# AI-Unicamp/interspeech_ser

Hardware: AMD Instinct MI355X
Metric: utterances/sec (10 s @16 kHz) WavLM-large embed extract (higher is better)
Workload: dtype bf16; 1 GPU; microsoft/wavlm-large embed extract, batch=16 x 10 s @16 kHz per GPU, all 25 hidden states to HBM, mode=bf16; a counted step = 8 such batches (128 utterances per GPU), 2 in flight at a time; batch=16, batches_in_flight=2, frames_per_utt=499, parallelism=utterance-sharded x1, no collective (one process)

## Files before the change

### interspeech_ser_amd/csrc/gemm.hip

```cpp
#include "ser_common.h"
#include "launch_plan.h"
#ifndef SER_GEMM_PP
#define SER_GEMM_PP 27
#endif
#include <stdlib.h>
#include <stdio.h>
#include <utility>
#ifdef SER_GEMM_DBG
extern "C" { void* ser_gemm_dbg_ptr = nullptr; }
__device__ unsigned long long* ser_gemm_dbg_dev = nullptr;
#endif

typedef const __attribute__((address_space(1))) void* gptr_t;
typedef __attribute__((address_space(3))) void* lptr_t;

__device__ __forceinline__ const char* uniform_ptr(const void* p) {
    const uint64_t v = (uint64_t)p;
    const uint32_t lo = __builtin_amdgcn_readfirstlane((uint32_t)v), hi = __builtin_amdgcn_readfirstlane((uint32_t)(v >> 32));
    return (const char*)(((uint64_t)hi << 32) | lo);
}
template <int BYTES>
__device__ __forceinline__ void dma_lds(const void* ubase, uint32_t voff, uint32_t lds_addr) {
    static_assert(BYTES == 16 || BYTES == 4, "dwordx4 or dword");
    if constexpr (BYTES == 16)
        asm volatile("s_mov_b32 m0, %2\n\tglobal_load_lds_dwordx4 %0, %1" :: "v"(voff), "s"(ubase), "s"(lds_addr) : "memory");
    else
        asm volatile("s_mov_b32 m0, %2\n\tglobal_load_lds_dword %0, %1" :: "v"(voff), "s"(ubase), "s"(lds_addr) : "memory");
}

template <int N>
__device__ __forceinline__ void wait_vmcnt() {
    if constexpr (N == 0) asm volatile("s_waitcnt vmcnt(0)" ::: "memory");
    else if constexpr (N == 1) asm volatile("s_waitcnt vmcnt(1)" ::: "memory");
    else if constexpr (N == 2) asm volatile("s_waitcnt vmcnt(2)" ::: "memory");
    else if constexpr (N == 3) asm volatile("s_waitcnt vmcnt(3)" ::: "memory");
    else if constexpr (N == 4) asm volatile("s_waitcnt vmcnt(4)" ::: "memory");
    else if constexpr (N == 5) asm volatile("s_waitcnt vmcnt(5)" ::: "memory");
    else if constexpr (N == 6) asm volatile("s_waitcnt vmcnt(6)" ::: "memory");
    else if constexpr (N == 7) asm volatile("s_waitcnt vmcnt(7)" ::: "memory");
    else if constexpr (N == 8) asm volatile("s_waitcnt vmcnt(8)" ::: "memory");
    else if constexpr (N == 10) asm volatile("s_waitcnt vmcnt(10)" ::: "memory");
    else if constexpr (N == 12) asm volatile("s_waitcnt vmcnt(12)" ::: "memory");
    else if constexpr (N == 16) asm volatile("s_waitcnt vmcnt(16)" ::: "memory");
    else static_assert(N < 0, "add a case");
}

__device__ __forceinline__ void mfma_scale8(f32x4& acc, const i32x8& a, const i32x8& b, int sa, int sb) {
    asm volatile("v_mfma_scale_f32_16x16x128_f8f6f4 %0, %1, %2, %0, %3, %4 op_sel_hi:[0,0,0]" : "+v"(acc) : "v"(a), "v"(b), "v"(sa), "v"(sb));
}
__device__ __forceinline__ void mfma_scale_drain() {
    asm volatile("s_nop 15\n\ts_nop 15\n\ts_nop 7" ::: "memory");
}

template <int WM, int WN, int TM, int TN, int BK, int ST, int MODE, bool LNEPI, int OM = MODE>
__global__ __launch_bounds__(64 * WM * WN, 2)
void ser_gemm_kernel(const ser_gemm_args p) {
    constexpr int NW = WM * WN, NT = 64 * NW;
    constexpr int BM = WM * TM * 16, BN = WN * TN * 16;
    constexpr int CH = BK / 8;
    constexpr int ROWB = BK * 2;
    constexpr int RPP = 1024 / ROWB;
    constexpr bool M16 = (MODE == SER_MODE_FP16M);
    constexpr int NPL = M16 ? 1 : mode_traits<MODE>::planes;
    constexpr int A_BYTES = BM * ROWB, W_BYTES = BN * ROWB, STAGE = NPL * (A_BYTES + W_BYTES);
    static_assert(!M16 || (BK == 64 && !LNEPI && (BM + BN) % 64 == 0), "FP16M: 64-deep K tiles, dense epilogue");
    constexpr int SCW = BM + BN;
    constexpr int LA = BM / RPP / NW, LW = BN / RPP / NW;
    constexpr int LPT = NPL * (LA + LW);
    constexpr int KS = BK / 32;
    static_assert(BM % (RPP * NW) == 0 && BN % (RPP * NW) == 0, "tile/wave mismatch");
    extern __shared__ __attribute__((aligned(16))) char lds[];

    const int tid = threadIdx.x;
    const int lane = tid & 63;
    const int wave = __builtin_amdgcn_readfirstlane(tid >> 6);
    const int wm = wave / WN, wn = wave % WN;
#ifdef SER_GEMM_DBG
    const unsigned long long dbg_e0 = __builtin_amdgcn_s_memtime();
#endif

    const int ntn = (p.N + BN - 1) / BN;
    const int ntm = (p.M + BM - 1) / BM;
    int bid = blockIdx.x;
    {
        const int nwg = ntm * ntn;
        const int q = nwg >> 3, r = nwg & 7, xcd = bid & 7;
        const int base = (xcd < r) ? xcd * (q + 1) : r * (q + 1) + (xcd - r) * q;
        bid = base + (bid >> 3);
    }
    const int mt = bid / ntn;
    const int nt = bid - mt * ntn;
    const int g = blockIdx.y;
    const int m0 = mt * BM, n0 = nt * BN;

    const unsigned short* Abase = (const unsigned short*)p.A + (int64_t)g * p.a_group_stride;
    const unsigned short* Wbase = (const unsigned short*)p.W + (int64_t)g * p.w_group_stride;

    const int prow = lane / CH, ppos = lane % CH;
    uint32_t aoff[LA], woff[LW];
    const int m0c = m0 < p.M ? m0 : p.M - 1;
    const int64_t arow0 = p.a_rowoff ? (int64_t)p.a_rowoff[m0c] * 8 : (int64_t)m0c * p.lda;
    const char* const Atile = uniform_ptr(Abase + arow0);
    const char* const Wtile = uniform_ptr(Wbase + (int64_t)n0 * p.K);
#pragma unroll
    for (int q = 0; q < LA; ++q) {
        const int R = (q * NW + wave) * RPP + prow;
        const int f = (BK == 64) ? (R & 7) : ((R >> 1) & 3);
        const int c = ppos ^ f;
        int m = m0 + R;
        m = m < p.M ? m : p.M - 1;
        const int64_t arow = p.a_rowoff ? (int64_t)p.a_rowoff[m] * 8 : (int64_t)m * p.lda;
        aoff[q] = (uint32_t)((arow - arow0 + c * 8) * 2);
    }
#pragma unroll
    for (int q = 0; q < LW; ++q) {
        const int R = (q * NW + wave) * RPP + prow;
        const int f = (BK == 64) ? (R & 7) : ((R >> 1) & 3);
        const int c = ppos ^ f;
        int n = n0 + R;
        n = n < p.N ? n : p.N - 1;
        woff[q] = (uint32_t)(((int64_t)(n - n0) * p.K + c * 8) * 2);
    }
    const uint32_t lds0 = __builtin_amdgcn_readfirstlane((uint32_t)(uintptr_t)(__attribute__((address_space(3))) char*)lds);

    const int nk = p.K / BK;
    const int total = M16 ? 2 * nk : nk;
    const int tpc = p.kc ? p.kc / BK : 0x7fffffff;

    unsigned char* const scl = (unsigned char*)(lds + ST * STAGE + (LNEPI ? 0 : BM * 8));
    const int sc_chunk = M16 ? (wave % (SCW / 64)) : 0;
    const bool sc_is_a = sc_chunk * 64 < BM;
    const char* const sc_base = uniform_ptr(sc_is_a ? p.a_scale : p.w_scale);
    const int64_t sc_step = (sc_is_a ? p.a_scale_ld : p.w_scale_ld) * 4;
    uint32_t sc_off = 0;
    if constexpr (M16) {
        const int r = sc_chunk * 64 + lane;
        int i = sc_is_a ? m0 + r : n0 + r - BM;
        const int lim = sc_is_a ? p.M : p.N;
        i = i < lim ? i : lim - 1;
        sc_off = (uint32_t)i * 4u;
    }
    int i_kk = 0, i_cc = 0, i_cj = 0, i_stage = 0;
    const char* is_ua = nullptr; const char* is_uw = nullptr;
    uint32_t is_dstA = 0, is_dstW = 0;
    auto issue_begin = [&]() {
        int64_t koffA = (int64_t)i_cj * p.ldj + (int64_t)i_cc * BK;
        int64_t koffW = (int64_t)i_kk * BK;
        if constexpr (M16) {
// ... 440 lines not shown
    if constexpr (LNEPI) {
        __syncthreads();
        float* red = (float*)lds;
        const float invN = 1.0f / (float)p.N;
        float mean[TM], rstd[TM], nmr[TM];
#pragma unroll
        for (int mi = 0; mi < TM; ++mi) {
            float s1 = 0.f, s2 = 0.f;
#pragma unroll
            for (int ni = 0; ni < TN; ++ni)
#pragma unroll
                for (int r = 0; r < 4; ++r) {
                    const float x = acc[ni][mi][r] + bias[ni * 4 + r];
                    acc[ni][mi][r] = x;
                    if (ncol0 + ni * 16 < p.N) { s1 += x; s2 += x * x; }
                }
            s1 += __shfl_xor(s1, 16, 64); s2 += __shfl_xor(s2, 16, 64);
            s1 += __shfl_xor(s1, 32, 64); s2 += __shfl_xor(s2, 32, 64);
            if (fq == 0) {
                red[((wm * TM * 16 + mi * 16 + frow) * WN + wn) * 2] = s1;
                red[((wm * TM * 16 + mi * 16 + frow) * WN + wn) * 2 + 1] = s2;
            }
        }
        __syncthreads();
#pragma unroll
        for (int mi = 0; mi < TM; ++mi) {
            float s1 = 0.f, s2 = 0.f;
#pragma unroll
            for (int w = 0; w < WN; ++w) {
                s1 += red[((wm * TM * 16 + mi * 16 + frow) * WN + w) * 2];
                s2 += red[((wm * TM * 16 + mi * 16 + frow) * WN + w) * 2 + 1];
            }
            mean[mi] = s1 * invN;
            rstd[mi] = rsqrtf(fmaxf(s2 * invN - mean[mi] * mean[mi], 0.f) + p.ln_eps);
            nmr[mi] = -mean[mi] * rstd[mi];
        }
        float lg[CPL], lb[CPL];
#pragma unroll
        for (int j4 = 0; j4 < TN; ++j4) {
            f32x4 a = {0.f, 0.f, 0.f, 0.f}, b = {0.f, 0.f, 0.f, 0.f};
            if (ncol0 + j4 * 16 < p.N) {
                a = *(const f32x4*)(p.ln_gamma + ncol0 + j4 * 16);
                b = *(const f32x4*)(p.ln_beta + ncol0 + j4 * 16);
            }
#pragma unroll
            for (int r = 0; r < 4; ++r) { lg[j4 * 4 + r] = a[r]; lb[j4 * 4 + r] = b[r]; }
        }
#pragma unroll
        for (int mi = 0; mi < TM; ++mi) {
            const int m = m0 + wm * TM * 16 + mi * 16 + frow;
            if (m >= p.M) continue;
            const int64_t orow = p.out_rowmap ? (int64_t)p.out_rowmap[m] : (int64_t)m;
#pragma unroll
            for (int ni = 0; ni < TN; ni += 2) {
                const bool ok0 = ncol0 + ni * 16 < p.N, ok1 = ncol0 + ni * 16 + 16 < p.N;
                float v[8];
#pragma unroll
                for (int r = 0; r < 8; ++r) {
                    const int nj = ni + (r >> 2), rr = r & 3;
                    v[r] = fmaf(fmaf(acc[nj][mi][rr], rstd[mi], nmr[mi]), lg[nj * 4 + rr], lb[nj * 4 + rr]);
                }
                if (p.act == SER_ACT_GELU) {
#pragma unroll
                    for (int r = 0; r < 8; r += 2) {
                        const f32x2 y = gelu2<MODE == SER_MODE_BF16>((f32x2){v[r], v[r + 1]});
                        v[r] = y[0]; v[r + 1] = y[1];
                    }
                }
                if (p.out_f32) {
                    f32x4 o0 = {v[0], v[1], v[2], v[3]}, o1 = {v[4], v[5], v[6], v[7]};
                    if (ok0) *(f32x4*)(p.out_f32 + (int64_t)m * p.ldo_f32 + gcol + ni * 16) = o0;
                    if (ok1) *(f32x4*)(p.out_f32 + (int64_t)m * p.ldo_f32 + gcol + ni * 16 + 16) = o1;
                }
                if (p.out_act) {
                    const int c8 = ni * 16 + ((fq & 1) ? 12 : 0);
                    store_act8_swap<MODE>((unsigned short*)p.out_act + orow * p.ldo_act + gcol + c8, p.out_plane_stride,
                                          ncol0 + c8 < p.N, v);
                    if constexpr (mode_traits<MODE>::f16) {
                        if (p.range_flag) range_fold8(ramax, v, ok0, ok1);
                    }
                }
            }
        }
    } else {
        const bool do_scale = p.col_scale_end > 0;
        const bool do_stat = p.stat_out != nullptr;
        float cs[TM];
#pragma unroll
        for (int mi = 0; mi < TM; ++mi) {
            cs[mi] = 0.f;
            if (p.shift_out) {
                int m = m0 + wm * TM * 16 + mi * 16 + frow;
                m = m < p.M ? m : p.M - 1;
                cs[mi] = p.shift_const + (p.shift_in ? p.shift_in[m] : 0.f);
            }
        }
        constexpr int RB = (TM * TN > 16) ? 2 : (TM < 4 ? TM : 4);
        f32x4 rres[RB][TN];
#pragma unroll
        for (int mi = 0; mi < TM; ++mi) {
            if (mi % RB == 0 && p.residual) {
#pragma unroll
                for (int u = 0; u < RB; ++u) {
                    int mr = m0 + wm * TM * 16 + (mi + u) * 16 + frow;
                    mr = mr < p.M ? mr : p.M - 1;
                    const int rr_ = p.res_row_mod ? (mr % p.res_row_mod) : mr;
#pragma unroll
                    for (int ni = 0; ni < TN; ++ni) {
                        f32x4 r = {0.f, 0.f, 0.f, 0.f};
                        if (ncol0 + ni * 16 < p.N) r = *(const f32x4*)(p.residual + (int64_t)rr_ * p.ldr + gcol + ni * 16);
                        rres[u][ni] = r;
                    }
                }
            }
            const int m = m0 + wm * TM * 16 + mi * 16 + frow;
            if (m >= p.M) continue;
            const int64_t orow = p.out_rowmap ? (int64_t)p.out_rowmap[m] : (int64_t)m;
            float mu = 0.f, rs = 1.f;
            if (p.ln_stats_in) {
                mu = lnst[2 * (wm * TM * 16 + mi * 16 + frow)];
                rs = lnst[2 * (wm * TM * 16 + mi * 16 + frow) + 1];
            }
            const float cshift = cs[mi];
            if (p.shift_out && nt == 0 && g == 0 && wn == 0 && fq == 0) p.shift_out[m] = cshift;
            const float* gsc = nullptr;
            const float* gsh = nullptr;
            if (p.gn_scale) {
                int lo = 0, hi = p.gn_B;
                while (hi - lo > 1) { const int mid = (lo + hi) >> 1; if (p.gn_row_offs[mid] <= m) lo = mid; else hi = mid; }
                gsc = p.gn_scale + (int64_t)lo * p.gn_ld + ncol0;
                gsh = p.gn_shift + (int64_t)lo * p.gn_ld + ncol0;
            }
            float st1 = 0.f, st2 = 0.f;
            unsigned mcode[2] = {0u, 0u};
#pragma unroll
            for (int ni = 0; ni < TN; ni += 2) {
                const bool ok0 = ncol0 + ni * 16 < p.N, ok1 = ncol0 + ni * 16 + 16 < p.N;
                float v[8];
#pragma unroll
                for (int r = 0; r < 8; ++r) {
                    const int nj = ni + (r >> 2), rr = r & 3;
                    float x = fmaf(rs, acc[nj][mi][rr] - mu * csum[nj * 4 + rr], bias[nj * 4 + rr]);
                    if (gsc && ncol0 + nj * 16 < p.N) x = fmaf(x, gsc[nj * 16 + rr], gsh[nj * 16 + rr]);
                    if (do_scale && ncol0 + nj * 16 < p.col_scale_end) x *= p.col_scale;
                    v[r] = x;
                }
                if (p.act == SER_ACT_GELU) {
#pragma unroll
                    for (int r = 0; r < 8; r += 2) {
                        const f32x2 y = gelu2<MODE == SER_MODE_BF16>((f32x2){v[r], v[r + 1]});
                        v[r] = y[0]; v[r + 1] = y[1];
                    }
                }
                if (p.residual) {
                    const f32x4 r0 = rres[mi % RB][ni], r1 = rres[mi % RB][ni + 1];
                    v[0] += r0[0]; v[1] += r0[1]; v[2] += r0[2]; v[3] += r0[3];
                    v[4] += r1[0]; v[5] += r1[1]; v[6] += r1[2]; v[7] += r1[3];
                }
                if (p.out_f32) {
                    float* op = p.out_f32 + (int64_t)m * p.ldo_f32 + gcol + ni * 16 - p.f32_col_begin;
                    f32x4 o0 = {v[0], v[1], v[2], v[3]}, o1 = {v[4], v[5], v[6], v[7]};
                    if (ok0 && ncol0 + ni * 16 >= p.f32_col_begin) *(f32x4*)op = o0;
                    if (ok1 && ncol0 + ni * 16 + 16 >= p.f32_col_begin) *(f32x4*)(op + 16) = o1;
                }
                if (p.shift_out) {
#pragma unroll
                    for (int r = 0; r < 8; ++r) v[r] -= cshift;
                }
                if (do_stat && ok0) {
#pragma unroll
                    for (int r = 0; r < 4; ++r) { st1 += v[r]; st2 += v[r] * v[r]; }
                }
                if (do_stat && ok1) {
#pragma unroll
                    for (int r = 4; r < 8; ++r) { st1 += v[r]; st2 += v[r] * v[r]; }
                }
                if (p.out_act) {
                    const int c8 = ni * 16 + ((fq & 1) ? 12 : 0);
                    if constexpr (OM == SER_MODE_FP16M) {
                        store_act8_swap<SER_MODE_FP16>((unsigned short*)p.out_act + orow * p.ldo_act + gcol + c8, 0, ncol0 + c8 < p.N, v);
                        float lo[8], ax = 0.f, al = 0.f;
#pragma unroll
                        for (int r = 0; r < 8; r += 2) {
                            const unsigned h2 = pack_h2(v[r], v[r + 1]);
                            lo[r] = v[r] - h2f((unsigned short)(h2 & 0xffffu));
                            lo[r + 1] = v[r + 1] - h2f((unsigned short)(h2 >> 16));
                            ax = fmaxf(ax, fmaxf(fabsf(v[r]), fabsf(v[r + 1])));
                            al = fmaxf(al, fmaxf(fabsf(lo[r]), fabsf(lo[r + 1])));
                        }
                        if (p.range_flag) range_fold8(ramax, v, ok0, ok1);
                        ax = max_rowquad(ax); al = max_rowquad(al);
                        const unsigned cx = mx_code(ax), cl = mx_code(al);
                        const float ix = mx_inv(cx), il = mx_inv(cl);
                        unsigned q4[4] = {mx_pack4(lo[0] * il, lo[1] * il, lo[2] * il, lo[3] * il), mx_pack4(lo[4] * il, lo[5] * il, lo[6] * il, lo[7] * il),
                                          mx_pack4(v[0] * ix, v[1] * ix, v[2] * ix, v[3] * ix), mx_pack4(v[4] * ix, v[5] * ix, v[6] * ix, v[7] * ix)};
                        transpose_rowquad(q4);
                        const int64_t bcol = gcol - fq * 4 + ni * 16;
                        unsigned char* seg = (unsigned char*)((unsigned short*)p.out_act + p.out_plane_stride) + (orow * p.ldo_act + (bcol & ~(int64_t)63)) * 2;
                        if (ok0) *(u32x4*)(seg + (fq >> 1) * 64 + (bcol & 63) + (fq & 1) * 16) = (u32x4){q4[0], q4[1], q4[2], q4[3]};
                        mcode[(ni >> 1) & 1] = cl | (cx << 16);
                        if (((ni >> 1) & 1) && fq == 0 && ok0)
                            p.out_scale[(bcol >> 6) * p.out_scale_ld + orow] = (mcode[0] & 0xffu) | ((mcode[1] & 0xffu) << 8) | (mcode[0] & 0xff0000u) | ((mcode[1] & 0xff0000u) << 8);
                    } else {
                        store_act8_swap<OM>((unsigned short*)p.out_act + orow * p.ldo_act + gcol + c8, p.out_plane_stride,
                                            ncol0 + c8 < p.N, v);
                        if constexpr (mode_traits<OM>::f16) {
                            if (p.range_flag) range_fold8(ramax, v, ok0, ok1);
                        }
                    }
                }
            }
            if (p.stat_out) {
                st1 += __shfl_xor(st1, 16, 64); st2 += __shfl_xor(st2, 16, 64);
                st1 += __shfl_xor(st1, 32, 64); st2 += __shfl_xor(st2, 32, 64);
                const int cstart = n0 + wn * (TN * 16);
                const int grp = g * ((p.N + 63) >> 6) + (cstart >> 6);
                if (fq == 0 && cstart < p.N && grp < p.stat_groups) {
                    float* d = p.stat_out + ((int64_t)m * p.stat_groups + grp) * 2;
                    d[0] = st1; d[1] = st2;
                    if constexpr (TN * 16 > 64) {
                        if (cstart + 64 < p.N) { d[2] = 0.f; d[3] = 0.f; }
                    }
                }
            }
        }
    }
    if constexpr (mode_traits<OM>::f16) range_report(p.range_flag, ramax);
#ifdef SER_GEMM_DBG
    {
        __builtin_amdgcn_sched_barrier(0);
        asm volatile("s_waitcnt vmcnt(0)" ::: "memory");
        const unsigned long long t2 = __builtin_amdgcn_s_memtime();
        unsigned long long* d = ser_gemm_dbg_dev;
        if (d && wave == 0 && lane == 0 && blockIdx.y == 0) d[131072 + blockIdx.x * 4 + 2] = t2;
    }
#endif
}

template <int... I, class F>
static bool with_index(int i, std::integer_sequence<int, I...>, F&& f) { return ser_with_mode<I...>(i, f); }

template <int TILE, int PAIR>
static int launch_planned(const ser_gemm_args* a, const gemm_launch& pl, hipStream_t s) {
    constexpr gemm_tile t = GEMM_TILE[TILE];
    constexpr gemm_pair pr = GEMM_PAIR[PAIR];
    auto k = ser_gemm_kernel<t.WM, t.WN, t.TM, t.TN, t.BK, t.ST, pr.mode, t.LNEPI, pr.om>;
    static std::atomic<bool> ready{false};
    if (pl.lds > 65536)
        if (hipError_t e = ser_lds_optin(k, pl.lds, ready)) return ser_fail((int)e, "ser_gemm: cannot raise dynamic LDS to %d", pl.lds);
    hipLaunchKernelGGL(k, dim3(pl.grid_x, pl.grid_y, 1), dim3((unsigned)pl.block, 1, 1), pl.lds, s, *a);
    return ser_check_launch("ser_gemm");
}

extern "C" int ser_gemm(const ser_gemm_args* a, void* stream) {
    gemm_launch pl;
    if (int rc = gemm_plan(a, &pl)) return rc;
    hipStream_t s = (hipStream_t)stream;
#ifdef SER_GEMM_DBG
    {
        static void* planted = nullptr;
        if (planted != ser_gemm_dbg_ptr) {
            planted = ser_gemm_dbg_ptr;
            (void)hipMemcpyToSymbol(HIP_SYMBOL(ser_gemm_dbg_dev), &planted, sizeof(void*));
        }
    }
#endif
    int rc = -22;
    with_index(pl.tile, std::make_integer_sequence<int, GEMM_TILES>{}, [&](auto T) {
        with_index(pl.pair, std::make_integer_sequence<int, GEMM_PAIRS>{}, [&](auto P) {
            constexpr int tile = decltype(T)::value, pair = decltype(P)::value;
            if constexpr (gemm_tile_serves(GEMM_TILE[tile], GEMM_PAIR[pair])) rc = launch_planned<tile, pair>(a, pl, s);
        });
    });
    return rc;
}
```

### interspeech_ser_amd/csrc/launch_plan.h

```cpp
#pragma once
#include <stddef.h>
#include <stdint.h>
#include <stdio.h>
#include <stdlib.h>
#include "../../include/ser_hip.h"

int ser_fail(int code, const char* fmt, ...);

#ifdef SER_EXPERIMENTS
static inline long ser_knob(const char* name, long dflt) { const char* e = getenv(name); return e ? atol(e) : dflt; }
#else
constexpr long ser_knob(const char*, long dflt) { return dflt; }
#endif

struct gemm_tile {
    const char* name;
    int WM, WN, TM, TN, BK, ST;
    bool LNEPI, two_plane;
    constexpr int BM() const { return WM * TM * 16; }
    constexpr int BN() const { return WN * TN * 16; }
    constexpr int threads() const { return 64 * WM * WN; }
    constexpr bool dense() const { return !LNEPI && BN() >= 128; }
};
enum gemm_tile_id {
// ... 33 lines not shown
constexpr int GEMM_PAIRS = (int)(sizeof(GEMM_PAIR) / sizeof(GEMM_PAIR[0]));
constexpr int gemm_pair_index(int mode, int om) {
    for (int i = 0; i < GEMM_PAIRS; ++i)
        if (GEMM_PAIR[i].mode == mode && GEMM_PAIR[i].om == om) return i;
    return -1;
}
constexpr bool gemm_two_plane(int mode) { return mode == SER_MODE_FP32X || mode == SER_MODE_FP16X; }
constexpr bool gemm_tile_serves(const gemm_tile& t, gemm_pair p) {
    if (t.two_plane != gemm_two_plane(p.mode)) return false;
    if (p.mode == SER_MODE_FP16M) return t.dense() && t.BK == 64;
    if (p.om == p.mode) return true;
    if (t.two_plane && p.om == SER_MODE_FP16) return !t.LNEPI;
    return t.dense();
}

struct gemm_knobs {
    int ln_bm, n64, deepk;
    long t256_min, x32_256_min, x32_sq_min, m16_sq_min, m16_256_min;
};
static inline const gemm_knobs& gemm_knobs_get() {
    static const gemm_knobs k = {
        (int)ser_knob("SER_GEMM_LN_BM", 0), (int)ser_knob("SER_GEMM_N64", 1), (int)ser_knob("SER_GEMM_DEEPK_256x128", 1),
        ser_knob("SER_GEMM_T256_MIN", 150),
        ser_knob("SER_GEMM_X32_256_MIN", 100),
        ser_knob("SER_GEMM_X32_SQ_MIN", 150), ser_knob("SER_GEMM_M16_SQ_MIN", 100), ser_knob("SER_GEMM_M16_256_MIN", 100)};
    return k;
}

#ifdef SER_EXPERIMENTS
static inline int gemm_forced_tile(const ser_gemm_args* a) {
    struct Rule { int n, k, cfg; };
    static Rule rules[8];
    static const int nrules = [] {
        const char* e = getenv("SER_GEMM_FORCE");
        int n = 0;
        while (e && *e && n < 8) {
            int a0, a1, a2, used = 0;
            if (sscanf(e, "%d:%d:%d%n", &a0, &a1, &a2, &used) != 3) break;
            rules[n++] = {a0, a1, a2};
            e += used;
            if (*e == ',') ++e;
        }
        return n;
    }();
    for (int i = 0; i < nrules; ++i)
        if (rules[i].n == a->N && rules[i].k == a->K && rules[i].cfg >= 0 && rules[i].cfg <= GEMM_256x256) return rules[i].cfg;
    return -1;
}
#endif

static inline int gemm_pick_tile(const ser_gemm_args* a) {
    const gemm_knobs& kn = gemm_knobs_get();
    const long rt256 = (a->M + 255) / 256;
    const long t256sq = rt256 * ((a->N + 255) / 256) * a->groups;
    const long t256x128 = rt256 * ((a->N + 127) / 128) * a->groups;
    if (gemm_two_plane(a->mode)) {
        if (a->ln_gamma) return GEMM_X_LN128x512x32;
        if (kn.n64 && a->N <= 64) return GEMM_X_128x64x32;
        const long sq_rounds = (t256sq + 255) / 256;
        const bool sq_full = t256sq * 100 >= sq_rounds * 256 * 85;
        if (kn.x32_sq_min > 0 && a->N >= 256 && t256sq >= kn.x32_sq_min && sq_full && a->act == SER_ACT_NONE) return GEMM_X_256x256x32;
        if (kn.x32_256_min > 0 && a->N >= 128 && t256x128 >= kn.x32_256_min) return GEMM_X_256x128x32;
        return GEMM_X_128x128x64;
    }
    if (a->mode == SER_MODE_FP16M) {
        if (a->tile_cfg == 3 || (!a->tile_cfg && a->N >= 256 && t256sq >= kn.m16_sq_min)) return GEMM_256x256;
        if (a->tile_cfg == 2 || (!a->tile_cfg && a->N >= 128 && t256x128 >= kn.m16_256_min)) return GEMM_256x128;
        return GEMM_128x128;
    }
    if (a->ln_gamma) {
        const int bm = kn.ln_bm ? kn.ln_bm : (a->M >= 200 * 128 ? 128 : (a->M >= 200 * 64 ? 64 : 32));
        return bm == 128 ? GEMM_LN512 : (bm == 64 ? GEMM_LN512_M64 : GEMM_LN512_M32);
    }
    if (a->tile_cfg > 0) return a->tile_cfg - 1;
#ifdef SER_EXPERIMENTS
    if (const int forced = gemm_forced_tile(a); forced >= 0) return forced;
#endif
    if (a->N >= 256 && t256sq >= kn.t256_min) return GEMM_256x256;
    if (kn.n64 && a->N <= 64) return GEMM_128x64;
    if (kn.deepk && a->groups == 1 && a->K >= 2048 && a->N >= 128 && a->M >= 512) return GEMM_256x128;
    return GEMM_128x128;
}

struct gemm_launch {
    int tile, pair;
    unsigned grid_x, grid_y;
    int block, lds;
};

static inline int gemm_plan(const ser_gemm_args* a, gemm_launch* out) {
    if (!a || !a->A || !a->W) return ser_fail(-1, "ser_gemm: null operand");
    if (a->M <= 0 || a->N <= 0 || a->K <= 0) return ser_fail(-2, "ser_gemm: bad shape M=%d N=%d K=%d", a->M, a->N, a->K);
    if (a->K % 64) return ser_fail(-3, "ser_gemm: K=%d must be a multiple of 64", a->K);
    if (a->kc && (a->kc % 64 || a->K % a->kc)) return ser_fail(-4, "ser_gemm: kc=%d must divide K and be a multiple of 64", a->kc);
    if (a->N % 8) return ser_fail(-5, "ser_gemm: N=%d must be a multiple of 8", a->N);
    if (gemm_pair_index(a->mode, a->mode) < 0) return ser_fail(-6, "ser_gemm: bad mode %d", a->mode);
    if (a->mode == SER_MODE_FP16M) {
        if (!a->a_scale || !a->w_scale || a->a_scale_ld < a->M || a->w_scale_ld < a->N)
            return ser_fail(-23, "ser_gemm: FP16M needs a_scale / w_scale with *_scale_ld >= the row count");
        if (a->a_rowoff || a->kc || a->groups != 1 || a->ln_gamma || (a->lda % 64))
            return ser_fail(-23, "ser_gemm: FP16M takes plain row-major operands (no row map / conv chunks / groups / LayerNorm epilogue), lda %% 64 == 0");
    }
    if (a->out_mode == SER_MODE_FP16M || (a->mode == SER_MODE_FP16M && !a->out_mode && a->out_act)) {
        if (!a->out_scale || (a->N % 64) || (a->ldo_act % 64) || a->groups != 1 || a->ln_gamma)
            return ser_fail(-24, "ser_gemm: an FP16M out_act needs out_scale, N %% 64 == 0, ldo_act %% 64 == 0, groups == 1, no LayerNorm epilogue");
    }
    if (!a->a_rowoff && (a->lda % 8)) return ser_fail(-7, "ser_gemm: lda must be a multiple of 8");
    if (a->groups < 1) return ser_fail(-8, "ser_gemm: groups=%d", a->groups);
    if (!a->out_f32 && !a->out_act) return ser_fail(-9, "ser_gemm: no output");
    if ((a->ldo_f32 % 4) || (a->ldo_act % 4) || (a->ldr % 4) || (a->c_group_stride % 4))
        return ser_fail(-10, "ser_gemm: output/residual pitches must be multiples of 4");
    if (a->ln_gamma) {
        if (!a->ln_beta) return ser_fail(-11, "ser_gemm: ln_gamma without ln_beta");
        if (a->N > 512 || a->groups != 1 || a->residual)
            return ser_fail(-12, "ser_gemm: the LayerNorm epilogue needs N <= 512, groups == 1, no residual");
    }
    if (a->ln_stats_in) {
        if (!a->ln_colsum || a->ln_groups < 2 || a->ln_groups > 32 || (a->ln_groups & 1) || a->ln_gamma)
            return ser_fail(-14, "ser_gemm: deferred LayerNorm needs ln_colsum, an even ln_groups in [2,32] and no fused-LN epilogue");
    }
    if (a->stat_out && (a->ln_gamma || a->stat_groups < a->groups * ((a->N + 63) / 64)))
        return ser_fail(-15, "ser_gemm: stat_out needs stat_groups >= groups*ceil(N/64) and no fused-LN epilogue");
    if (a->shift_out && (!a->stat_out || a->ln_gamma)) return ser_fail(-19, "ser_gemm: shift_out needs stat_out and no fused-LN epilogue");
    if (a->mean_out && !a->ln_stats_in) return ser_fail(-20, "ser_gemm: mean_out needs ln_stats_in");
    if (a->lnstat_out && !a->ln_stats_in) return ser_fail(-20, "ser_gemm: lnstat_out needs ln_stats_in");
    const int om = a->out_mode ? a->out_mode : a->mode;
    const int pair = gemm_pair_index(a->mode, om);
    if (om != a->mode && !a->ln_gamma && pair < 0)
        return ser_fail(-21, "ser_gemm: out_mode %d with mode %d (FP32X -> FP16, FP16 <-> FP16X, FP16X <-> FP16M convert)", a->out_mode, a->mode);
    if (om != a->mode && a->ln_gamma) return ser_fail(-21, "ser_gemm: out_mode %d with the LayerNorm epilogue", a->out_mode);
    if (a->col_scale_end % 4) return ser_fail(-17, "ser_gemm: col_scale_end must be a multiple of 4");
    if (a->gn_scale && (!a->gn_shift || !a->gn_row_offs || a->gn_B < 1 || a->gn_ld < a->N || (a->gn_ld % 4) || a->groups != 1 ||
                        a->ln_gamma || a->ln_stats_in))
        return ser_fail(-25, "ser_gemm: gn_scale needs gn_shift, gn_row_offs, gn_B >= 1, gn_ld >= N (multiple of 4), groups == 1, "
                             "no LayerNorm epilogue and no deferred LayerNorm");
    if ((a->ldo_act % 8) || (a->c_group_stride % 8)) return ser_fail(-18, "ser_gemm: act pitch / group stride must be multiples of 8");
    if (a->f32_col_begin < 0 || (a->f32_col_begin % 8)) return ser_fail(-16, "ser_gemm: f32_col_begin must be a non-negative multiple of 8");
    if (a->tile_cfg < 0 || a->tile_cfg > 3) return ser_fail(-13, "ser_gemm: tile_cfg=%d (0 auto, 1..3)", a->tile_cfg);

    const int tile = gemm_pick_tile(a);
    const gemm_tile& t = GEMM_TILE[tile];
    if (!gemm_tile_serves(t, GEMM_PAIR[pair])) {
        if (a->mode == SER_MODE_FP16M) return ser_fail(-22, "ser_gemm: FP16M needs a dense tile (N > 64, no LayerNorm epilogue)");
        if (a->mode == SER_MODE_FP16X) return ser_fail(-22, "ser_gemm: FP16X -> FP16M output needs a dense tile (N > 64)");
        return ser_fail(-22, "ser_gemm: FP16 -> FP16X output needs a dense tile (N > 64, no LayerNorm epilogue)");
    }
    const int BM = t.BM(), BN = t.BN();
    out->tile = tile;
    out->pair = pair;
    out->grid_x = (unsigned)(((a->M + BM - 1) / BM) * ((a->N + BN - 1) / BN));
    out->grid_y = (unsigned)a->groups;
    out->block = t.threads();
    out->lds = (gemm_two_plane(a->mode) ? 2 : 1) * t.ST * (BM + BN) * t.BK * 2 + (t.LNEPI ? 0 : BM * 8)
             + (a->mode == SER_MODE_FP16M ? t.ST * (BM + BN) * 4 : 0);
    return 0;
}

constexpr int ATTN_BKV = 64;
constexpr int ATTN_NWV = 4;

struct attn_launch {
    int dhp, mode;
    bool pre, tbl, b2d, gb, occ;
    int nbuf, bias_stride;
    size_t lds;
    int nq;
    unsigned grid;
};
constexpr int attn_qk_planes(int mode) { return (mode == SER_MODE_FP32X || mode == SER_MODE_FP16X || mode == SER_MODE_FP16Q) ? 2 : 1; }
constexpr int attn_v_planes(int mode) { return (mode == SER_MODE_FP32X || mode == SER_MODE_FP16X) ? 2 : 1; }
constexpr bool attn_form_built(int dhp, int mode, bool pre, bool tbl, bool b2d, bool gb, bool occ) {
    if (b2d) return dhp == 64 && pre && !tbl && !gb && !occ && (mode == SER_MODE_BF16 || mode == SER_MODE_FP32X || mode == SER_MODE_FP16X);
    if (gb) return dhp == 64 && pre && tbl && !occ;
    if (occ) return dhp == 64 && attn_qk_planes(mode) == 1;
    return pre || (mode != SER_MODE_FP16X && mode != SER_MODE_FP16Q);
}

static inline int attn_plan(const ser_attention_args* a, attn_launch* out) {
    if (!a) return ser_fail(-1, "ser_attention: null pointer");
    if (!a->qkv || !a->frame_offs || !a->out) return ser_fail(-1, "ser_attention: null pointer");
    const int np = attn_qk_planes(a->mode), npv = attn_v_planes(a->mode);
    if (a->gate_x) {
        if (!a->table || !a->gru_const || a->gate || !a->gate_stat || !a->gate_w || !a->gate_cb)
            return ser_fail(-13, "ser_attention: gate_x needs table, gru_const, gate_stat, gate_w, gate_cb and no gate[]");
        if ((a->gate_x_ld % 8) || (a->gate_x_plane_stride % 8) || (a->gate_w_plane_stride % 8) || a->gate_x_planes != np || (a->dh % 8))
            return ser_fail(-13, "ser_attention: gate_x / gate_w pitch, or gate_x_planes != the planes of mode %d", a->mode);
    }
    if (a->out_mode && a->out_mode != SER_MODE_FP16M) return ser_fail(-14, "ser_attention: out_mode %d (0 or SER_MODE_FP16M)", a->out_mode);
    if (a->out_mode == SER_MODE_FP16M &&
        (a->mode != SER_MODE_FP16X || a->dh != 64 || !a->out_scale || (a->ldo % 64) || a->bias2d || a->out_scale_ld <= 0))
        return ser_fail(-14, "ser_attention: SER_MODE_FP16M context rows need mode FP16X, head dim 64, out_scale, ldo %% 64 == 0 and no bias2d");
    if (a->B <= 0 || a->H <= 0 || a->max_frames <= 0) return ser_fail(-2, "ser_attention: bad B/H/max_frames");
    if (a->dh % 8 || a->dh < 8 || a->dh > 128) return ser_fail(-3, "ser_attention: head dim %d unsupported (multiple of 8, <= 128)", a->dh);
    if ((a->ld % 8) || (a->ldo % 4) || (a->q_col % 8) || (a->k_col % 8) || (a->v_col % 8)) return ser_fail(-4, "ser_attention: misaligned pitches/columns");
    if (a->mode < SER_MODE_BF16 || a->mode > SER_MODE_FP16Q) return ser_fail(-5, "ser_attention: bad mode %d", a->mode);
    if ((a->table != nullptr) != (a->gate != nullptr || a->gru_const != nullptr))
        return ser_fail(-6, "ser_attention: the bias table needs a gate (gate[] or gate_col + gru_const) and vice versa");
    if (a->gate && a->gru_const) return ser_fail(-9, "ser_attention: give gate[] or gru_const, not both");
    if (a->gru_const && !a->gate_x && (a->gate_col < 0 || (a->gate_col % 2))) return ser_fail(-10, "ser_attention: bad gate_col %d", a->gate_col);
    if (a->table && a->table_T < a->max_frames) return ser_fail(-7, "ser_attention: bias table built for T=%d < max_frames=%d", a->table_T, a->max_frames);
    const bool pre = a->scale <= 0.f;
    if (a->bias2d) {
        if (a->table || !a->key_lens || !pre || a->dh > 64 || a->mode == SER_MODE_FP16 || a->mode == SER_MODE_FP16Q)
            return ser_fail(-11, "ser_attention: bias2d needs key_lens, a pre-scaled q (scale <= 0), dh <= 64, no table, bf16 / fp32x / fp16x");
        if (a->bias2d_ld < a->max_frames || (a->bias2d_ld % ATTN_BKV))
            return ser_fail(-12, "ser_attention: bias2d_ld=%lld must be a multiple of %d and >= max_frames", (long long)a->bias2d_ld, ATTN_BKV);
    }
    const int dhp = a->dh <= 64 ? 64 : (a->dh <= 96 ? 96 : 128);
    const int nch = ATTN_BKV * (dhp / 8) / (64 * ATTN_NWV);
    const int nq = (a->max_frames + 32 * ATTN_NWV - 1) / (32 * ATTN_NWV);
    const unsigned nblocks = (unsigned)(((a->H * a->B + 7) / 8) * 8 * nq);
    int bias_stride = 0;
    if (a->table) {
        bias_stride = ((a->max_frames + 32 * ATTN_NWV + 2 * ATTN_BKV + 3 + 4) / 4) * 4;
        bias_stride += (16 - (bias_stride & 63) + 64) & 63;
    }
    const auto nbuf_of = [&](bool occ_) { return (!occ_ && nch * (np + npv) <= 8) ? 2 : 1; };
    const auto lds_of = [&](int nbuf_) { return (size_t)nbuf_ * (np + npv) * ATTN_BKV * dhp * 2 + (size_t)4 * bias_stride * 4; };
    bool occ = dhp == 64 && np == 1 && !a->bias2d && nblocks > 2u * 256u && nblocks <= 4u * 256u;
    int nbuf = nbuf_of(occ);
    size_t lds = lds_of(nbuf);
    if (occ && lds > 40 * 1024) {
        occ = false;
        nbuf = nbuf_of(occ);
        lds = lds_of(nbuf);
    }
    const bool gb = a->table && lds > 160 * 1024 && pre && dhp == 64 && ATTN_NWV == 4;
    if (gb) {
        occ = false;
        nbuf = nbuf_of(occ);
        bias_stride = 0;
        lds = lds_of(nbuf);
// ... 8 lines not shown
```

### interspeech_ser_amd/csrc/launch_plan_check.cc

```cpp
#include "launch_plan.h"
#include <string.h>
#include <iostream>
#include <sstream>
#include <string>

enum kind { I32, I64, F32, PTR };
struct field { const char* name; size_t off; kind k; };
#define F(S, M, K) {#M, offsetof(S, M), K}
static const field GEMM_FIELDS[] = {
    F(ser_gemm_args, A, PTR), F(ser_gemm_args, a_rowoff, PTR), F(ser_gemm_args, lda, I64), F(ser_gemm_args, kc, I32), F(ser_gemm_args, W, PTR),
    F(ser_gemm_args, M, I32), F(ser_gemm_args, N, I32), F(ser_gemm_args, K, I32), F(ser_gemm_args, groups, I32),
    F(ser_gemm_args, c_group_stride, I32), F(ser_gemm_args, mode, I32), F(ser_gemm_args, act, I32), F(ser_gemm_args, residual, PTR),
    F(ser_gemm_args, ldr, I64), F(ser_gemm_args, out_f32, PTR), F(ser_gemm_args, ldo_f32, I64), F(ser_gemm_args, out_act, PTR),
    F(ser_gemm_args, ldo_act, I64), F(ser_gemm_args, ln_gamma, PTR), F(ser_gemm_args, ln_beta, PTR), F(ser_gemm_args, tile_cfg, I32),
    F(ser_gemm_args, ln_stats_in, PTR), F(ser_gemm_args, ln_groups, I32), F(ser_gemm_args, ln_colsum, PTR), F(ser_gemm_args, stat_out, PTR),
    F(ser_gemm_args, stat_groups, I32), F(ser_gemm_args, f32_col_begin, I32), F(ser_gemm_args, col_scale_end, I32),
    F(ser_gemm_args, shift_out, PTR), F(ser_gemm_args, out_mode, I32), F(ser_gemm_args, mean_out, PTR), F(ser_gemm_args, lnstat_out, PTR),
    F(ser_gemm_args, a_scale, PTR), F(ser_gemm_args, a_scale_ld, I64), F(ser_gemm_args, w_scale, PTR), F(ser_gemm_args, w_scale_ld, I64),
    F(ser_gemm_args, out_scale, PTR), F(ser_gemm_args, gn_scale, PTR), F(ser_gemm_args, gn_shift, PTR), F(ser_gemm_args, gn_row_offs, PTR),
    F(ser_gemm_args, gn_B, I32), F(ser_gemm_args, gn_ld, I32),
};
static const field ATTN_FIELDS[] = {
    F(ser_attention_args, qkv, PTR), F(ser_attention_args, ld, I64), F(ser_attention_args, q_col, I32), F(ser_attention_args, k_col, I32),
    F(ser_attention_args, v_col, I32), F(ser_attention_args, B, I32), F(ser_attention_args, frame_offs, PTR), F(ser_attention_args, table, PTR),
    F(ser_attention_args, gate, PTR), F(ser_attention_args, max_frames, I32), F(ser_attention_args, table_T, I32), F(ser_attention_args, out, PTR),
    F(ser_attention_args, ldo, I64), F(ser_attention_args, H, I32), F(ser_attention_args, dh, I32), F(ser_attention_args, scale, F32),
    F(ser_attention_args, mode, I32), F(ser_attention_args, gate_col, I32), F(ser_attention_args, out_mode, I32),
    F(ser_attention_args, gru_const, PTR), F(ser_attention_args, key_lens, PTR), F(ser_attention_args, bias2d, PTR),
    F(ser_attention_args, bias2d_ld, I64), F(ser_attention_args, gate_x, PTR), F(ser_attention_args, gate_x_ld, I64),
    F(ser_attention_args, gate_x_plane_stride, I64), F(ser_attention_args, gate_stat, PTR), F(ser_attention_args, gate_w, PTR),
    F(ser_attention_args, gate_cb, PTR), F(ser_attention_args, gate_x_planes, I32), F(ser_attention_args, gate_w_plane_stride, I64),
    F(ser_attention_args, out_scale, PTR), F(ser_attention_args, out_scale_ld, I64),
};
#undef F

static char g_dummy[16];

template <size_t N>
static bool parse(std::istringstream& in, void* args, const field (&fields)[N]) {
    std::string tok;
    while (in >> tok) {
        const size_t eq = tok.find('=');
        if (eq == std::string::npos) return false;
        const std::string name = tok.substr(0, eq), val = tok.substr(eq + 1);
        const field* f = nullptr;
        for (const field& c : fields)
            if (name == c.name) f = &c;
        if (!f) return false;
        char* dst = (char*)args + f->off;
        switch (f->k) {
            case I32: { const int32_t v = (int32_t)strtol(val.c_str(), nullptr, 10); memcpy(dst, &v, sizeof(v)); break; }
            case I64: { const int64_t v = (int64_t)strtoll(val.c_str(), nullptr, 10); memcpy(dst, &v, sizeof(v)); break; }
            case F32: { const float v = strtof(val.c_str(), nullptr); memcpy(dst, &v, sizeof(v)); break; }
            case PTR: { const void* v = val == "0" ? nullptr : g_dummy; memcpy(dst, &v, sizeof(v)); break; }
        }
    }
    return true;
}

int main() {
    std::string line;
    int lineno = 0;
    while (std::getline(std::cin, line)) {
        ++lineno;
        std::istringstream in(line);
        std::string what;
        if (!(in >> what)) continue;
        bool ok = false;
        if (what == "gemm") {
            ser_gemm_args a = {};
            gemm_launch pl = {};
            if ((ok = parse(in, &a, GEMM_FIELDS))) {
                const int rc = gemm_plan(&a, &pl);
                if (rc) printf("gemm err %d\n", rc);
                else printf("gemm %s %d>%d grid=%ux%u block=%d lds=%d\n", GEMM_TILE[pl.tile].name, GEMM_PAIR[pl.pair].mode, GEMM_PAIR[pl.pair].om,
                            pl.grid_x, pl.grid_y, pl.block, pl.lds);
            }
        } else if (what == "attn") {
            ser_attention_args a = {};
            attn_launch pl = {};
            if ((ok = parse(in, &a, ATTN_FIELDS))) {
                const int rc = attn_plan(&a, &pl);
                if (rc) printf("attn err %d\n", rc);
                else printf("attn %d %d %c%c%c%c%c nbuf=%d bias_stride=%d lds=%zu grid=%u\n", pl.dhp, pl.mode, pl.pre ? 'P' : '-', pl.tbl ? 'T' : '-',
                            pl.b2d ? 'B' : '-', pl.gb ? 'G' : '-', pl.occ ? 'O' : '-', pl.nbuf, pl.bias_stride, pl.lds, pl.grid);
            }
        }
        if (!ok) {
            fprintf(stderr, "launch_plan_check: cannot read line %d: %s\n", lineno, line.c_str());
            return 2;
        }
    }
    return 0;
}
```

Baseline: 2055 utterances/s.

## Add specialized GEMM epilogue variants for LN-activation and residual outputs

Adds a template parameter selecting a specialized epilogue class (LN+activation, or residual add with f32 output) alongside the generic one. The planner picks a specialized epilogue when the argument flags match, and inside it GELU and column-scale choices are resolved into compile-time branches per tile. The aim is to cut runtime branching and register pressure in the generic epilogue for the common transformer GEMMs. In exchange it adds more kernel instantiations, so binary size and compile time grow, and there is a risk of mismatched behaviour if the selection conditions are incomplete.

After: 2169 utterances/s (median of 6 runs). 1.06x the previous value.

```diff
diff --git a/interspeech_ser_amd/csrc/gemm.hip b/interspeech_ser_amd/csrc/gemm.hip
--- a/interspeech_ser_amd/csrc/gemm.hip
+++ b/interspeech_ser_amd/csrc/gemm.hip
@@ -52,7 +52,7 @@
     asm volatile("s_nop 15\n\ts_nop 15\n\ts_nop 7" ::: "memory");
 }
 
-template <int WM, int WN, int TM, int TN, int BK, int ST, int MODE, bool LNEPI, int OM = MODE>
+template <int WM, int WN, int TM, int TN, int BK, int ST, int MODE, bool LNEPI, int OM = MODE, int EPI = GEMM_EPI_GENERIC>
 __global__ __launch_bounds__(64 * WM * WN, 2)
 void ser_gemm_kernel(const ser_gemm_args p) {
     constexpr int NW = WM * WN, NT = 64 * NW;
@@ -64,6 +64,7 @@
     constexpr int NPL = M16 ? 1 : mode_traits<MODE>::planes;
     constexpr int A_BYTES = BM * ROWB, W_BYTES = BN * ROWB, STAGE = NPL * (A_BYTES + W_BYTES);
     static_assert(!M16 || (BK == 64 && !LNEPI && (BM + BN) % 64 == 0), "FP16M: 64-deep K tiles, dense epilogue");
+    static_assert(EPI == GEMM_EPI_GENERIC || !LNEPI, "epilogue classes: dense epilogue only");
     constexpr int SCW = BM + BN;
     constexpr int LA = BM / RPP / NW, LW = BN / RPP / NW;
     constexpr int LPT = NPL * (LA + LW);
@@ -670,7 +671,7 @@
                 }
             }
         }
-    } else {
+    } else if constexpr (EPI == GEMM_EPI_GENERIC) {
         const bool do_scale = p.col_scale_end > 0;
         const bool do_stat = p.stat_out != nullptr;
         float cs[TM];
@@ -812,6 +813,165 @@
                 }
             }
         }
+    } else {
+        constexpr bool LNA = EPI == GEMM_EPI_LN_ACT, RES = EPI == GEMM_EPI_RESID;
+        static_assert(LNA || RES, "epilogue class");
+        int ncol_e = ncol0;
+        asm volatile("" : "+v"(ncol_e));
+        const int64_t gcol = (int64_t)g * p.c_group_stride + ncol_e;
+        const bool do_scale = p.col_scale_end > 0;
+        const bool f_copy = LNA || p.out_act;
+        const bool f_shift = RES && p.shift_out;
+        const bool do_stat = RES && p.stat_out != nullptr;
+        float cs[TM];
+#pragma unroll
+        for (int mi = 0; mi < TM; ++mi) {
+            cs[mi] = 0.f;
+            if (f_shift) {
+                int m = m0 + wm * TM * 16 + mi * 16 + frow;
+                m = m < p.M ? m : p.M - 1;
+                cs[mi] = p.shift_const + (p.shift_in ? p.shift_in[m] : 0.f);
+            }
+        }
+        constexpr int RB = (TM * TN > 16) ? 2 : (TM < 4 ? TM : 4);
+        auto rows = [&](auto act_tag, auto scl_tag) {
+            constexpr int ACT = decltype(act_tag)::value, SCL = decltype(scl_tag)::value;
+            f32x4 rres[RB][TN];
+#pragma unroll
+            for (int mi = 0; mi < TM; ++mi) {
+                if (RES && mi % RB == 0) {
+#pragma unroll
+                    for (int u = 0; u < RB; ++u) {
+                        int mr = m0 + wm * TM * 16 + (mi + u) * 16 + frow;
+                        mr = mr < p.M ? mr : p.M - 1;
+                        const int rr_ = p.res_row_mod ? (mr % p.res_row_mod) : mr;
+#pragma unroll
+                        for (int ni = 0; ni < TN; ++ni) {
+                            f32x4 r = {0.f, 0.f, 0.f, 0.f};
+                            if (ncol0 + ni * 16 < p.N) r = *(const f32x4*)(p.residual + (int64_t)rr_ * p.ldr + gcol + ni * 16);
+                            rres[u][ni] = r;
+                        }
+                    }
+                }
+                const int m = m0 + wm * TM * 16 + mi * 16 + frow;
+                if (m >= p.M) continue;
+                const int64_t orow = p.out_rowmap ? (int64_t)p.out_rowmap[m] : (int64_t)m;
+                float mu = 0.f, rs = 1.f;
+                if (LNA) {
+                    mu = lnst[2 * (wm * TM * 16 + mi * 16 + frow)];
+                    rs = lnst[2 * (wm * TM * 16 + mi * 16 + frow) + 1];
+                }
+                const float cshift = cs[mi];
+                if (f_shift && nt == 0 && g == 0 && wn == 0 && fq == 0) p.shift_out[m] = cshift;
+                float* const f32row = RES ? p.out_f32 + (int64_t)m * p.ldo_f32 + gcol : nullptr;
+                unsigned short* const actrow = f_copy ? (unsigned short*)p.out_act + orow * p.ldo_act + gcol : nullptr;
+                float st1 = 0.f, st2 = 0.f;
+                unsigned mcode[2] = {0u, 0u};
+#pragma unroll
+                for (int ni = 0; ni < TN; ni += 2) {
+                    const bool ok0 = ncol0 + ni * 16 < p.N, ok1 = ncol0 + ni * 16 + 16 < p.N;
+                    float v[8];
+#pragma unroll
+                    for (int r = 0; r < 8; ++r) {
+                        const int nj = ni + (r >> 2), rr = r & 3;
+                        float x = RES ? acc[nj][mi][rr] + bias[nj * 4 + rr] : fmaf(rs, acc[nj][mi][rr] - mu * csum[nj * 4 + rr], bias[nj * 4 + rr]);
+                        if (SCL == 2 && do_scale && ncol0 + nj * 16 < p.col_scale_end) x *= p.col_scale;
+                        if constexpr (SCL == 1) {
+                            x *= p.col_scale;
+                            asm("" : "+v"(x));
+                        }
+                        v[r] = x;
+                    }
+                    if (ACT == 1 || (ACT == 2 && p.act == SER_ACT_GELU)) {
+#pragma unroll
+                        for (int r = 0; r < 8; r += 2) {
+                            const f32x2 y = gelu2<MODE == SER_MODE_BF16>((f32x2){v[r], v[r + 1]});
+                            v[r] = y[0]; v[r + 1] = y[1];
+                        }
+                    }
+                    if constexpr (RES) {
+                        const f32x4 r0 = rres[mi % RB][ni], r1 = rres[mi % RB][ni + 1];
+                        v[0] += r0[0]; v[1] += r0[1]; v[2] += r0[2]; v[3] += r0[3];
+                        v[4] += r1[0]; v[5] += r1[1]; v[6] += r1[2]; v[7] += r1[3];
+                    }
+                    if constexpr (RES) {
+                        float* op = f32row + ni * 16;
+                        f32x4 o0 = {v[0], v[1], v[2], v[3]}, o1 = {v[4], v[5], v[6], v[7]};
+                        if (ok0) *(f32x4*)op = o0;
+                        if (ok1) *(f32x4*)(op + 16) = o1;
+                    }
+                    if (f_shift) {
+#pragma unroll
+                        for (int r = 0; r < 8; ++r) v[r] -= cshift;
+                    }
+                    if (do_stat && ok0) {
+#pragma unroll
+                        for (int r = 0; r < 4; ++r) { st1 += v[r]; st2 += v[r] * v[r]; }
+                    }
+                    if (do_stat && ok1) {
+#pragma unroll
+                        for (int r = 4; r < 8; ++r) { st1 += v[r]; st2 += v[r] * v[r]; }
+                    }
+                    if (f_copy) {
+                        const int c8 = ni * 16 + ((fq & 1) ? 12 : 0);
+                        if constexpr (OM == SER_MODE_FP16M) {
+                            store_act8_swap<SER_MODE_FP16>(actrow + c8, 0, ncol0 + c8 < p.N, v);
+                            float lo[8], ax = 0.f, al = 0.f;
+#pragma unroll
+                            for (int r = 0; r < 8; r += 2) {
+                                const unsigned h2 = pack_h2(v[r], v[r + 1]);
+                                lo[r] = v[r] - h2f((unsigned short)(h2 & 0xffffu));
+                                lo[r + 1] = v[r + 1] - h2f((unsigned short)(h2 >> 16));
+                                ax = fmaxf(ax, fmaxf(fabsf(v[r]), fabsf(v[r + 1])));
+                                al = fmaxf(al, fmaxf(fabsf(lo[r]), fabsf(lo[r + 1])));
+                            }
+                            if (p.range_flag) range_fold8(ramax, v, ok0, ok1);
+                            ax = max_rowquad(ax); al = max_rowquad(al);
+                            const unsigned cx = mx_code(ax), cl = mx_code(al);
+                            const float ix = mx_inv(cx), il = mx_inv(cl);
+                            unsigned q4[4] = {mx_pack4(lo[0] * il, lo[1] * il, lo[2] * il, lo[3] * il), mx_pack4(lo[4] * il, lo[5] * il, lo[6] * il, lo[7] * il),
+                                              mx_pack4(v[0] * ix, v[1] * ix, v[2] * ix, v[3] * ix), mx_pack4(v[4] * ix, v[5] * ix, v[6] * ix, v[7] * ix)};
+                            transpose_rowquad(q4);
+                            const int64_t bcol = gcol - fq * 4 + ni * 16;
+                            unsigned char* seg = (unsigned char*)((unsigned short*)p.out_act + p.out_plane_stride) + (orow * p.ldo_act + (bcol & ~(int64_t)63)) * 2;
+                            if (ok0) *(u32x4*)(seg + (fq >> 1) * 64 + (bcol & 63) + (fq & 1) * 16) = (u32x4){q4[0], q4[1], q4[2], q4[3]};
+                            mcode[(ni >> 1) & 1] = cl | (cx << 16);
+                            if (((ni >> 1) & 1) && fq == 0 && ok0)
+                                p.out_scale[(bcol >> 6) * p.out_scale_ld + orow] = (mcode[0] & 0xffu) | ((mcode[1] & 0xffu) << 8) | (mcode[0] & 0xff0000u) | ((mcode[1] & 0xff0000u) << 8);
+                        } else {
+                            store_act8_swap<OM>(actrow + c8, p.out_plane_stride, ncol0 + c8 < p.N, v);
+                            if constexpr (mode_traits<OM>::f16) {
+                                if (p.range_flag) range_fold8(ramax, v, ok0, ok1);
+                            }
+                        }
+                    }
+                }
+                if (do_stat) {
+                    st1 += __shfl_xor(st1, 16, 64); st2 += __shfl_xor(st2, 16, 64);
+                    st1 += __shfl_xor(st1, 32, 64); st2 += __shfl_xor(st2, 32, 64);
+                    const int cstart = n0 + wn * (TN * 16);
+                    const int grp = g * ((p.N + 63) >> 6) + (cstart >> 6);
+                    if (fq == 0 && cstart < p.N && grp < p.stat_groups) {
+                        float* d = p.stat_out + ((int64_t)m * p.stat_groups + grp) * 2;
+                        d[0] = st1; d[1] = st2;
+                        if constexpr (TN * 16 > 64) {
+                            if (cstart + 64 < p.N) { d[2] = 0.f; d[3] = 0.f; }
+                        }
+                    }
+                }
+            }
+        };
+        using std::integral_constant;
+        if constexpr (LNA) {
+            const bool gelu = p.act == SER_ACT_GELU;
+            const bool scl_all = n0 + BN <= p.col_scale_end, scl_none = p.col_scale_end <= n0;
+            if (gelu && scl_none) rows(integral_constant<int, 1>{}, integral_constant<int, 0>{});
+            else if (!gelu && scl_all) rows(integral_constant<int, 0>{}, integral_constant<int, 1>{});
+            else if (!gelu && scl_none) rows(integral_constant<int, 0>{}, integral_constant<int, 0>{});
+            else rows(integral_constant<int, 2>{}, integral_constant<int, 2>{});
+        } else {
+            rows(integral_constant<int, 0>{}, integral_constant<int, 0>{});
+        }
     }
     if constexpr (mode_traits<OM>::f16) range_report(p.range_flag, ramax);
 #ifdef SER_GEMM_DBG
@@ -828,11 +988,11 @@
 template <int... I, class F>
 static bool with_index(int i, std::integer_sequence<int, I...>, F&& f) { return ser_with_mode<I...>(i, f); }
 
-template <int TILE, int PAIR>
+template <int TILE, int PAIR, int EPI>
 static int launch_planned(const ser_gemm_args* a, const gemm_launch& pl, hipStream_t s) {
     constexpr gemm_tile t = GEMM_TILE[TILE];
     constexpr gemm_pair pr = GEMM_PAIR[PAIR];
-    auto k = ser_gemm_kernel<t.WM, t.WN, t.TM, t.TN, t.BK, t.ST, pr.mode, t.LNEPI, pr.om>;
+    auto k = ser_gemm_kernel<t.WM, t.WN, t.TM, t.TN, t.BK, t.ST, pr.mode, t.LNEPI, pr.om, EPI>;
     static std::atomic<bool> ready{false};
     if (pl.lds > 65536)
         if (hipError_t e = ser_lds_optin(k, pl.lds, ready)) return ser_fail((int)e, "ser_gemm: cannot raise dynamic LDS to %d", pl.lds);
@@ -857,7 +1017,10 @@
     with_index(pl.tile, std::make_integer_sequence<int, GEMM_TILES>{}, [&](auto T) {
         with_index(pl.pair, std::make_integer_sequence<int, GEMM_PAIRS>{}, [&](auto P) {
             constexpr int tile = decltype(T)::value, pair = decltype(P)::value;
-            if constexpr (gemm_tile_serves(GEMM_TILE[tile], GEMM_PAIR[pair])) rc = launch_planned<tile, pair>(a, pl, s);
+            with_index(pl.epi, std::make_integer_sequence<int, GEMM_EPIS>{}, [&](auto E) {
+                constexpr int epi = decltype(E)::value;
+                if constexpr (gemm_epi_built(tile, GEMM_PAIR[pair], epi)) rc = launch_planned<tile, pair, epi>(a, pl, s);
+            });
         });
     });
     return rc;
diff --git a/interspeech_ser_amd/csrc/launch_plan.h b/interspeech_ser_amd/csrc/launch_plan.h
--- a/interspeech_ser_amd/csrc/launch_plan.h
+++ b/interspeech_ser_amd/csrc/launch_plan.h
@@ -139,10 +139,27 @@
     return GEMM_128x128;
 }
 
+enum gemm_epi_id { GEMM_EPI_GENERIC, GEMM_EPI_LN_ACT, GEMM_EPI_RESID, GEMM_EPIS };
+constexpr const char* GEMM_EPI_NAME[GEMM_EPIS] = {"GENERIC", "LN_ACT", "RESID"};
+constexpr bool gemm_epi_built(int tile, gemm_pair p, int epi) {
+    if (epi == GEMM_EPI_GENERIC) return gemm_tile_serves(GEMM_TILE[tile], p);
+    if (tile != GEMM_128x128 && tile != GEMM_256x128 && tile != GEMM_256x256) return false;
+    if (!gemm_tile_serves(GEMM_TILE[tile], p) || gemm_two_plane(p.mode)) return false;
+    return epi == GEMM_EPI_RESID || !(p.mode == SER_MODE_FP16 && p.om == SER_MODE_FP16X);
+}
+static inline int gemm_pick_epi(const ser_gemm_args* a, int tile, int pair) {
+    int epi = GEMM_EPI_GENERIC;
+    if (a->gn_scale) return epi;
+    if (a->ln_stats_in && a->out_act && !a->residual && !a->out_f32 && !a->shift_out && !a->stat_out) epi = GEMM_EPI_LN_ACT;
+    else if (a->residual && a->out_f32 && !a->f32_col_begin && a->col_scale_end <= 0 && !a->ln_stats_in && a->act != SER_ACT_GELU) epi = GEMM_EPI_RESID;
+    return gemm_epi_built(tile, GEMM_PAIR[pair], epi) ? epi : GEMM_EPI_GENERIC;
+}
+
 struct gemm_launch {
     int tile, pair;
     unsigned grid_x, grid_y;
     int block, lds;
+    int epi;
 };
 
 static inline int gemm_plan(const ser_gemm_args* a, gemm_launch* out) {
@@ -205,6 +222,7 @@
     const int BM = t.BM(), BN = t.BN();
     out->tile = tile;
     out->pair = pair;
+    out->epi = gemm_pick_epi(a, tile, pair);
     out->grid_x = (unsigned)(((a->M + BM - 1) / BM) * ((a->N + BN - 1) / BN));
     out->grid_y = (unsigned)a->groups;
     out->block = t.threads();
diff --git a/interspeech_ser_amd/csrc/launch_plan_check.cc b/interspeech_ser_amd/csrc/launch_plan_check.cc
--- a/interspeech_ser_amd/csrc/launch_plan_check.cc
+++ b/interspeech_ser_amd/csrc/launch_plan_check.cc
@@ -58,7 +58,8 @@
     return true;
 }
 
-int main() {
+int main(int argc, char** argv) {
+    const bool show_epi = argc > 1 && !strcmp(argv[1], "--epi");
     std::string line;
     int lineno = 0;
     while (std::getline(std::cin, line)) {
@@ -73,8 +74,11 @@
             if ((ok = parse(in, &a, GEMM_FIELDS))) {
                 const int rc = gemm_plan(&a, &pl);
                 if (rc) printf("gemm err %d\n", rc);
-                else printf("gemm %s %d>%d grid=%ux%u block=%d lds=%d\n", GEMM_TILE[pl.tile].name, GEMM_PAIR[pl.pair].mode, GEMM_PAIR[pl.pair].om,
-                            pl.grid_x, pl.grid_y, pl.block, pl.lds);
+                else {
+                    printf("gemm %s %d>%d grid=%ux%u block=%d lds=%d", GEMM_TILE[pl.tile].name, GEMM_PAIR[pl.pair].mode, GEMM_PAIR[pl.pair].om,
+                           pl.grid_x, pl.grid_y, pl.block, pl.lds);
+                    printf(show_epi ? " epi=%s\n" : "\n", GEMM_EPI_NAME[pl.epi]);
+                }
             }
         } else if (what == "attn") {
             ser_attention_args a = {};
```
